# daigo0927/pwcnet

Hardware: AMD Instinct MI355X
Metric: image_pairs_per_sec_448x1024 (higher is better)
Workload: dtype f32 via fp16x2-split MFMA (fp32 tensors and accumulation; big stride-1 convs, level-1 extractor and correlation on the F16 pipe)

## Files before the change

### pwcnet_amd/csrc/conv3x3_h2.hip

```cpp
#pragma once
#include "pwc_common.h"
#include <type_traits>

typedef float pwc_f32x16 __attribute__((ext_vector_type(16)));

struct H2Args {
    const float* x;
    const void* wp;
    const float* bias;
    float* y;
    int x_cs, y_cs;
    int N, H, W;
    int Cin_phys, Cout;
    int apply_act;
    float slope;
    int tiles_x, tiles_y, ncb;
    int dil_y, dil_x;
    int ntiles;
    float* ws_partial;
    unsigned* dbg;
    int Ho, Wo;
    const float* x2;
    int x2_cs, nc16_a;
    const float* x3;
// ... 583 lines not shown
    const H2Geo geo = h2_geometry(H, W, dilation, Cout);
    const int hs = geo.hs, ws = geo.ws;
    const bool filled = nb >= 192 || (nb >= 64 && h2_split_pays(nb, Cin_phys >> 4, h2_cu_count()));
    return hs >= 7 && ws >= 24 && filled && Cin_phys >= 32 ? 1 : 0;
}

#ifdef PWC_HARNESS
static unsigned* h2_debug_counters = nullptr;
#else
constexpr unsigned* h2_debug_counters = nullptr;
#endif

template <int CT, int PT, int WCG, int ABL, int XS = 1, bool S2 = false>
static int h2_launch(H2Args& a, int hs, int ws, float* workspace, size_t workspace_floats, hipStream_t stream) {
    typedef H2Cfg<CT, PT, WCG, XS> C;
    a.tiles_x = (ws + 31) / 32; a.tiles_y = (hs + C::TR - 1) / C::TR; a.ncb = a.Cout / (32 * C::NCT);
    const long nblk = (long)a.N * a.dil_y * a.dil_x * a.tiles_x * a.tiles_y * a.ncb;
    if (nblk * (a.Cin_phys >> 4) >= (1L << 31)) return PWC_ERANGE;
    a.ntiles = (int)nblk;
    const int cus = h2_cu_count();
    int grid = a.ntiles;
    a.ws_partial = nullptr;
    const size_t part = (size_t)C::NCT * 32 * C::TR * 32;
    if (workspace && h2_split_pays(a.ntiles, a.Cin_phys >> 4, cus) && workspace_floats >= (size_t)cus * part) {
        grid = cus;
        a.ws_partial = workspace;
    }
    pwc_allow_dynamic_lds<&conv3x3_h2_kernel<CT, PT, WCG, ABL, XS, S2>>(C::LDS);
    hipLaunchKernelGGL((conv3x3_h2_kernel<CT, PT, WCG, ABL, XS, S2>), dim3((unsigned)grid), dim3(512), C::LDS, stream, a);
    return pwc_launch_status();
}

static bool h2s2_tile_routed(int N, int H, int W, int x_cs, int Cin_phys, int Cout) {
    const bool ok = h2s2_has_tile_image(Cin_phys, Cout) && pwc_conv3x3_s2_tile_admits(N, H, W, x_cs, Cin_phys, Cout);
#ifdef PWC_HARNESS
    if (pwc_conv3x3_s2_tile_debug_mode()) return ok && pwc_conv3x3_s2_tile_debug_mode() > 0;
#endif
    return ok && Cin_phys == 32;
}

template <int ABL = 0>
static int h2_run(const float* x, int x_cs, const float* packed_w, const float* bias, float* y, int y_cs, int N, int H, int W,
                  int Cin_phys, int Cout, int dilation, int apply_act, float slope, pwc_stream_t stream, int variant = 0,
                  float* workspace = nullptr, size_t workspace_floats = 0, int stride = 1, const float* x2 = nullptr, int x2_cs = 0,
                  int Cin_a_phys = 0, uint32_t* status = nullptr, const float* x3 = nullptr, int x3_cs = 0, int Cin_b_phys = 0) {
    if (!x || !packed_w || !bias || !y) return PWC_EINVAL;
    if (x3 && !x2) return PWC_EINVAL;
    const int slack = x3 ? 12 : 0;
    if (x2) {
        const int cb = x3 ? Cin_b_phys : Cin_phys - Cin_a_phys;
        if (Cin_a_phys <= 0 || Cin_a_phys >= Cin_phys || (Cin_a_phys % 16) || x_cs < Cin_a_phys - slack || x2_cs < cb - slack) return PWC_EINVAL;
        if ((x2_cs & 3) || !pwc_aligned16(x2)) return PWC_EALIGN;
        if ((long)H * W * x2_cs * 4 >= (long)PWC_OOB) return PWC_ERANGE;
    }
    if (x3) {
        const int cc = Cin_phys - Cin_a_phys - Cin_b_phys;
        if (Cin_b_phys <= 0 || (Cin_b_phys % 16) || cc <= 0 || x3_cs < cc - 12 || dilation != 1) return PWC_EINVAL;
        if ((x3_cs & 3) || !pwc_aligned16(x3)) return PWC_EALIGN;
        if ((long)H * W * x3_cs * 4 >= (long)PWC_OOB) return PWC_ERANGE;
    }
    if (reinterpret_cast<uintptr_t>(status) & 7u) return PWC_EALIGN;
    if (dilation < 1 || (stride != 1 && stride != 2)) return PWC_EINVAL;
    const bool shape_ok = !(Cin_phys % 16 || Cout % 32 || Cout > H2_MAX_COUT || (stride == 2 && (dilation != 1 || (H & 1) || (W & 1) || x2)));
    if (const int rc = pwc_conv_io_check(x, x_cs, x2 ? Cin_a_phys - slack : Cin_phys, y, y_cs, Cout, packed_w, bias, N, H, W, shape_ok)) return rc;
    if (!pwc_aligned16(workspace)) return PWC_EALIGN;
    if (((long)H * W + W + 2) * x_cs * 4 >= (long)PWC_OOB || (long)H * W * y_cs * 4 >= (long)PWC_OOB) return PWC_ERANGE;
    H2Args a;
    a.x = x; a.wp = packed_w; a.bias = bias; a.y = y; a.x_cs = x_cs; a.y_cs = y_cs;
    a.N = N; a.H = H; a.W = W; a.Cin_phys = Cin_phys; a.Cout = Cout; a.apply_act = apply_act; a.slope = slope;
    const bool s2 = stride == 2;
    a.Ho = s2 ? H / 2 : H; a.Wo = s2 ? W / 2 : W;
    if (s2) a.Cin_phys = 4 * Cin_phys;
    const H2Geo geo = h2_geometry(a.Ho, a.Wo, dilation, Cout);
    a.dil_y = geo.dy; a.dil_x = geo.dx;
    a.dbg = h2_debug_counters;
    a.x2 = x2; a.x2_cs = x2_cs; a.nc16_a = x2 ? Cin_a_phys >> 4 : a.Cin_phys >> 4; a.status = status;
    a.x3 = x3; a.x3_cs = x3_cs; a.nc16_b = x3 ? Cin_b_phys >> 4 : (a.Cin_phys >> 4) - a.nc16_a;
    const int hs = geo.hs, ws = geo.ws;
    if (variant == 0) variant = h2_plan(N, a.Ho, a.Wo, a.Cin_phys, Cout, dilation, nullptr);
    if (variant < 1 || variant > 5) return PWC_EUNSUPPORTED;
    if (Cout % h2_variant(variant).couts) return PWC_EUNSUPPORTED;
    if (s2 && h2s2_tile_routed(N, H, W, x_cs, Cin_phys, Cout))
        return pwc_conv3x3_s2_tile_launch(x, x_cs, packed_w + h2s2_tile_image_offset(Cin_phys, Cout), bias, y, y_cs, N, H, W, Cin_phys,
                                          Cout, apply_act, slope, stream);
    if (s2) {
        switch (variant) {
            case 1: return h2_launch<2, 2, 2, ABL, 1, true>(a, hs, ws, workspace, workspace_floats, (hipStream_t)stream);
            case 2: return h2_launch<2, 2, 1, ABL, 1, true>(a, hs, ws, workspace, workspace_floats, (hipStream_t)stream);
            case 3: return h2_launch<3, 1, 1, ABL, 1, true>(a, hs, ws, workspace, workspace_floats, (hipStream_t)stream);
            case 4: return h2_launch<1, 2, 1, ABL, 1, true>(a, hs, ws, workspace, workspace_floats, (hipStream_t)stream);
            default: return h2_launch<1, 2, 2, ABL, 1, true>(a, hs, ws, workspace, workspace_floats, (hipStream_t)stream);
        }
    }
    if (geo.xs == 2) {
        switch (variant) {
            case 1: return h2_launch<2, 2, 2, ABL, 2>(a, hs, ws, workspace, workspace_floats, (hipStream_t)stream);
            case 3: return h2_launch<3, 1, 1, ABL, 2>(a, hs, ws, workspace, workspace_floats, (hipStream_t)stream);
            case 5: return h2_launch<1, 2, 2, ABL, 2>(a, hs, ws, workspace, workspace_floats, (hipStream_t)stream);
            default: return PWC_EUNSUPPORTED;
        }
    }
    switch (variant) {
        case 1: return h2_launch<2, 2, 2, ABL>(a, hs, ws, workspace, workspace_floats, (hipStream_t)stream);
        case 2: return h2_launch<2, 2, 1, ABL>(a, hs, ws, workspace, workspace_floats, (hipStream_t)stream);
        case 3: return h2_launch<3, 1, 1, ABL>(a, hs, ws, workspace, workspace_floats, (hipStream_t)stream);
        case 4: return h2_launch<1, 2, 1, ABL>(a, hs, ws, workspace, workspace_floats, (hipStream_t)stream);
        default: return h2_launch<1, 2, 2, ABL>(a, hs, ws, workspace, workspace_floats, (hipStream_t)stream);
    }
}

extern "C" size_t pwc_conv3x3_h2_workspace_floats(int N, int H, int W, int Cin_phys, int Cout, int dilation) {
    long nb = 0;
    const int v = h2_plan(N, H, W, Cin_phys, Cout, dilation, &nb);
    const int cus = h2_cu_count();
    if (!v || !h2_split_pays(nb, Cin_phys >> 4, cus)) return 0;
    const H2Variant t = h2_variant(v);
    return (size_t)cus * t.couts * t.rows * 32;
}

extern "C" int pwc_conv3x3_h2_f32(const float* x, int x_cs, const float* packed_w, const float* bias, float* y,
                                  int y_cs, int N, int H, int W, int Cin_phys, int Cout, int dilation,
                                  int apply_act, float slope, float* workspace, size_t workspace_floats, pwc_stream_t stream) {
    return h2_run<0>(x, x_cs, packed_w, bias, y, y_cs, N, H, W, Cin_phys, Cout, dilation, apply_act, slope, stream, 0,
                     workspace, workspace_floats);
}

extern "C" int pwc_conv3x3_h2_ex_f32(const float* x, int x_cs, int Cin_a_phys, const float* x2, int x2_cs,
                                     const float* packed_w, const float* bias, float* y, int y_cs, int N, int H, int W,
                                     int Cin_phys, int Cout, int dilation, int apply_act, float slope, float* workspace,
                                     size_t workspace_floats, uint32_t* status, pwc_stream_t stream) {
    return h2_run<0>(x, x_cs, packed_w, bias, y, y_cs, N, H, W, Cin_phys, Cout, dilation, apply_act, slope, stream, 0,
                     workspace, workspace_floats, 1, x2, x2_cs, Cin_a_phys, status);
}

extern "C" int pwc_conv3x3_h2_ex3_f32(const float* x, int x_cs, int Cin_a_phys, const float* x2, int x2_cs, int Cin_b_phys,
                                      const float* x3, int x3_cs, const float* packed_w, const float* bias, float* y, int y_cs,
                                      int N, int H, int W, int Cin_phys, int Cout, int apply_act, float slope, float* workspace,
                                      size_t workspace_floats, uint32_t* status, pwc_stream_t stream) {
    if (!x2 || !x3) return PWC_EINVAL;
    return h2_run<0>(x, x_cs, packed_w, bias, y, y_cs, N, H, W, Cin_phys, Cout, 1, apply_act, slope, stream, 0,
                     workspace, workspace_floats, 1, x2, x2_cs, Cin_a_phys, status, x3, x3_cs, Cin_b_phys);
}

extern "C" int pwc_conv3x3_h2_stride2_supported(int N, int H, int W, int Cin_phys, int Cout) {
    if (H <= 0 || W <= 0 || (H & 1) || (W & 1) || Cin_phys % 16 || Cin_phys > 32) return 0;
    return pwc_conv3x3_h2_supported(N, H / 2, W / 2, 4 * Cin_phys, Cout, 1);
}

extern "C" size_t pwc_conv3x3_h2_stride2_workspace_floats(int N, int H, int W, int Cin_phys, int Cout) {
    if ((H & 1) || (W & 1)) return 0;
    return pwc_conv3x3_h2_workspace_floats(N, H / 2, W / 2, 4 * Cin_phys, Cout, 1);
}

extern "C" int pwc_conv3x3_h2_stride2_f32(const float* x, int x_cs, const float* packed_w, const float* bias, float* y,
                                          int y_cs, int N, int H, int W, int Cin_phys, int Cout, int apply_act, float slope,
                                          float* workspace, size_t workspace_floats, uint32_t* status, pwc_stream_t stream) {
    return h2_run<0>(x, x_cs, packed_w, bias, y, y_cs, N, H, W, Cin_phys, Cout, 1, apply_act, slope, stream, 0,
                     workspace, workspace_floats, 2, nullptr, 0, 0, status);
}

extern "C" int pwc_conv3x3_h2_plan(int N, int H, int W, int Cin_phys, int Cout, int dilation) {
    return h2_plan(N, H, W, Cin_phys, Cout, dilation, nullptr);
}

extern "C" int pwc_conv3x3_h2_variant_f32(const float* x, int x_cs, const float* packed_w, const float* bias, float* y,
                                          int y_cs, int N, int H, int W, int Cin_phys, int Cout, int dilation,
                                          int apply_act, float slope, int variant, float* workspace, size_t workspace_floats,
// ... 6 lines not shown
```

### pwcnet_amd/csrc/conv3x3_s2.hip

```cpp
#include "pwc_common.h"

typedef unsigned int s2_u32x4 __attribute__((ext_vector_type(4)));
#define S2_OOB 0x80000000u

constexpr int S2_PC = 2 * PWC_S2_TILE_COLS + 1;
constexpr int S2_PR = 2 * PWC_S2_TILE_ROWS + 1;
constexpr int S2_NPX = S2_PR * S2_PC;
constexpr int S2_EVEN = PWC_S2_TILE_COLS + 1;
constexpr int S2_LINE = S2_PC * 32;
constexpr int S2_CC = 64;
constexpr int S2_UB = 5;

struct S2Args {
    const float* x;
    const float* wp;
    const float* bias;
    float* y;
    int x_cs, y_cs;
    int N, H, W, Ho, Wo;
    int Cin_phys, Cout;
    int pad_t, pad_l;
    int apply_act;
    float slope;
    int ntx, nty;
    int cg;
    int nsteps;
};

template <int NBW>
__global__ __launch_bounds__(512) void conv3x3_s2_kernel(const S2Args a) {
    extern __shared__ __attribute__((aligned(16))) char s2_smem[];
    const int t = threadIdx.x, lane = t & 63;
    const int wave = __builtin_amdgcn_readfirstlane(t >> 6);
    int b = blockIdx.x;
    const int tx = b % a.ntx;
    b /= a.ntx;
    const int ty = b % a.nty, n = b / a.nty;

    const __amdgpu_buffer_rsrc_t rx = __builtin_amdgcn_make_buffer_rsrc(
        (void*)a.x, 0, (int)((size_t)a.N * a.H * a.W * a.x_cs * 4), 0x00020000);
    const __amdgpu_buffer_rsrc_t rw = __builtin_amdgcn_make_buffer_rsrc(
        (void*)a.wp, 0, (int)((size_t)a.Cout * a.nsteps * 128), 0x00020000);
    const int m = lane & 15, kq = lane >> 4;
    const int row = wave >> 1, cb0 = (wave & 1) * NBW, nb = a.Cout >> 4;

    f32x4 hh[2][NBW], xx[2][NBW];
#pragma unroll
    for (int hf = 0; hf < 2; ++hf)
#pragma unroll
        for (int j = 0; j < NBW; ++j) {
            hh[hf][j] = f32x4{0.f, 0.f, 0.f, 0.f};
            xx[hf][j] = f32x4{0.f, 0.f, 0.f, 0.f};
        }

    auto fetch_b = [&](s2_u32x4 (&bv)[NBW][2], int s, bool live) {
#pragma unroll
        for (int j = 0; j < NBW; ++j) {
            const int cb = cb0 + j;
            const unsigned vo = (live && cb < nb) ? (unsigned)((cb * a.nsteps + s) * 2048 + lane * 16) : S2_OOB;
            bv[j][0] = __builtin_amdgcn_raw_buffer_load_b128(rw, (int)vo, 0, 0);
            bv[j][1] = __builtin_amdgcn_raw_buffer_load_b128(rw, (int)vo, 1024, 0);
        }
    };

    const int gy0 = 2 * PWC_S2_TILE_ROWS * ty - a.pad_t, gx0 = 2 * PWC_S2_TILE_COLS * tx - a.pad_l;
    for (int c0 = 0; c0 < a.Cin_phys; c0 += S2_CC) {
        const int cc = a.Cin_phys - c0 < S2_CC ? a.Cin_phys - c0 : S2_CC;
        const int cgc = cc >> 5, ng16 = cc >> 4, cqs = 1 + cgc;
        const int nst = 9 * cgc, sbase = c0 >> 5;
        auto gstep = [&](int si) { const int tap = si / cgc; return tap * a.cg + sbase + (si - tap * cgc); };
        if (c0) __syncthreads();
        s2_u32x4 b0[NBW][2], b1[NBW][2];
        fetch_b(b0, gstep(0), true);
        const int nu = S2_NPX << cqs;
#pragma unroll 1
        for (int u0 = t; u0 < nu; u0 += 512 * S2_UB) {
            f32x4 v[S2_UB][2];
            int dst[S2_UB];
#pragma unroll
            for (int k = 0; k < S2_UB; ++k) {
                const int u = u0 + 512 * k;
                const int px = u >> cqs, j = u - (px << cqs);
                const int pr = px / S2_PC, pc = px - pr * S2_PC;
                const int gy = gy0 + pr, gx = gx0 + pc;
                const bool ok = u < nu && (unsigned)gy < (unsigned)a.H && (unsigned)gx < (unsigned)a.W;
                const unsigned vo = ok ? (unsigned)(((n * a.H + gy) * a.W + gx) * a.x_cs + c0 + j * 8) * 4u : S2_OOB;
                v[k][0] = __builtin_bit_cast(f32x4, __builtin_amdgcn_raw_buffer_load_b128(rx, (int)vo, 0, 0));
                v[k][1] = __builtin_bit_cast(f32x4, __builtin_amdgcn_raw_buffer_load_b128(rx, (int)vo, 16, 0));
                const int pos = (pc & 1) ? S2_EVEN + (pc >> 1) : pc >> 1;
                dst[k] = u < nu ? ((pr * ng16 + (j >> 1)) * 2) * S2_LINE + pos * 32 + (j & 1) * 16 : -1;
            }
#pragma unroll
            for (int k = 0; k < S2_UB; ++k)
                if (dst[k] >= 0) {
                    pwc_f16x4 h0, m0, h1, m1;
                    pwc_split4(v[k][0], h0, m0);
                    pwc_split4(v[k][1], h1, m1);
                    *reinterpret_cast<pwc_f16x8*>(s2_smem + dst[k]) = __builtin_shufflevector(h0, h1, 0, 1, 2, 3, 4, 5, 6, 7);
                    *reinterpret_cast<pwc_f16x8*>(s2_smem + dst[k] + S2_LINE) = __builtin_shufflevector(m0, m1, 0, 1, 2, 3, 4, 5, 6, 7);
                }
        }
        __syncthreads();

        auto step = [&](const s2_u32x4 (&bv)[NBW][2], int si) {
            const int tap = si / cgc, c32 = si - tap * cgc;
            const int dy = tap / 3, dx = tap - 3 * dy;
            const int pos = (dx == 1 ? S2_EVEN : 0) + (dx >> 1) + m;
            const char* p = s2_smem + (((2 * row + dy) * ng16 + 2 * c32 + (kq >> 1)) * 2) * S2_LINE + pos * 32 + (kq & 1) * 16;
            pwc_f16x8 ah[2], am[2];
#pragma unroll
            for (int hf = 0; hf < 2; ++hf) {
                ah[hf] = *reinterpret_cast<const pwc_f16x8*>(p + hf * 512);
                am[hf] = *reinterpret_cast<const pwc_f16x8*>(p + hf * 512 + S2_LINE);
            }
#pragma unroll
            for (int j = 0; j < NBW; ++j) {
                const pwc_f16x8 wh = __builtin_bit_cast(pwc_f16x8, bv[j][0]);
                const pwc_f16x8 wm = __builtin_bit_cast(pwc_f16x8, bv[j][1]);
#pragma unroll
                for (int hf = 0; hf < 2; ++hf) {
                    xx[hf][j] = __builtin_amdgcn_mfma_f32_16x16x32_f16(wm, ah[hf], xx[hf][j], 0, 0, 0);
                    hh[hf][j] = __builtin_amdgcn_mfma_f32_16x16x32_f16(wh, ah[hf], hh[hf][j], 0, 0, 0);
                    xx[hf][j] = __builtin_amdgcn_mfma_f32_16x16x32_f16(wh, am[hf], xx[hf][j], 0, 0, 0);
                }
            }
        };
#pragma unroll 1
        for (int si = 0; si < nst; si += 2) {
            fetch_b(b1, gstep(si + 1 < nst ? si + 1 : 0), si + 1 < nst);
            step(b0, si);
            fetch_b(b0, gstep(si + 2 < nst ? si + 2 : 0), si + 2 < nst);
            if (si + 1 < nst) step(b1, si + 1);
        }
    }

    const int oy = PWC_S2_TILE_ROWS * ty + row;
#pragma unroll
    for (int hf = 0; hf < 2; ++hf) {
        const int ox = PWC_S2_TILE_COLS * tx + hf * 16 + m;
        if (oy < a.Ho && ox < a.Wo) {
            float* yp = a.y + ((size_t)(n * a.Ho + oy) * a.Wo + ox) * a.y_cs + 4 * kq;
#pragma unroll
            for (int j = 0; j < NBW; ++j) {
                const int cb = cb0 + j;
                if (cb < nb) {
                    f32x4 v = __builtin_elementwise_fma(xx[hf][j], f32x4{1.f / 2048.f, 1.f / 2048.f, 1.f / 2048.f, 1.f / 2048.f}, hh[hf][j]);
                    v += *reinterpret_cast<const f32x4*>(a.bias + cb * 16 + 4 * kq);
                    if (a.apply_act) v = pwc_lrelu4(v, a.slope);
                    *reinterpret_cast<f32x4*>(yp + cb * 16) = v;
                }
            }
        }
    }
}

template <int NBW>
static int s2_launch(const S2Args& a, hipStream_t s) {
    const long wgs = (long)a.N * a.nty * a.ntx;
    if (wgs >= (1L << 31)) return PWC_ERANGE;
    const int cc = a.Cin_phys < S2_CC ? a.Cin_phys : S2_CC;
    pwc_allow_dynamic_lds<&conv3x3_s2_kernel<NBW>>(S2_NPX * S2_CC * 4);
    hipLaunchKernelGGL((conv3x3_s2_kernel<NBW>), dim3((unsigned)wgs), dim3(512), (size_t)S2_NPX * cc * 4, s, a);
    return pwc_launch_status();
}

bool pwc_conv3x3_s2_tile_admits(int N, int H, int W, int x_cs, int Cin_phys, int Cout) {
    if (N <= 0 || H <= 0 || W <= 0 || Cin_phys <= 0 || Cout <= 0 || x_cs < Cin_phys) return false;
    if (Cin_phys % 32 || Cout % 16 || Cout > 128) return false;
    return pwc_fits_2g(N, H, W, x_cs) && (long)Cout * 9 * (Cin_phys / 32) * 128 < (1L << 31);
}

long pwc_conv3x3_s2_tile_count(int N, int H, int W) {
    const int Ho = (H + 1) / 2, Wo = (W + 1) / 2;
    return (long)N * ((Ho + PWC_S2_TILE_ROWS - 1) / PWC_S2_TILE_ROWS) * ((Wo + PWC_S2_TILE_COLS - 1) / PWC_S2_TILE_COLS);
}

int pwc_conv3x3_s2_tile_launch(const float* x, int x_cs, const float* packed_w, const float* bias, float* y, int y_cs, int N, int H,
                               int W, int Cin_phys, int Cout, int apply_act, float slope, pwc_stream_t stream) {
    if (!pwc_conv3x3_s2_tile_admits(N, H, W, x_cs, Cin_phys, Cout)) return PWC_EUNSUPPORTED;
    S2Args a;
    a.x = x; a.wp = packed_w; a.bias = bias; a.y = y; a.x_cs = x_cs; a.y_cs = y_cs;
    a.N = N; a.H = H; a.W = W;
    pwc_same_pad(H, 2, 1, &a.Ho, &a.pad_t);
    pwc_same_pad(W, 2, 1, &a.Wo, &a.pad_l);
    a.Cin_phys = Cin_phys; a.Cout = Cout; a.apply_act = apply_act; a.slope = slope;
    a.ntx = (a.Wo + PWC_S2_TILE_COLS - 1) / PWC_S2_TILE_COLS;
    a.nty = (a.Ho + PWC_S2_TILE_ROWS - 1) / PWC_S2_TILE_ROWS;
    a.cg = Cin_phys / 32; a.nsteps = 9 * a.cg;
    hipStream_t s = (hipStream_t)stream;
    switch ((Cout / 16 + 1) / 2) {
        case 1: return s2_launch<1>(a, s);
        case 2: return s2_launch<2>(a, s);
        case 3: return s2_launch<3>(a, s);
        default: return s2_launch<4>(a, s);
    }
}

#ifdef PWC_HARNESS
static int s2_tile_mode = 0;
extern "C" int pwc_debug_conv3x3_s2_tile(int mode) { s2_tile_mode = mode; return 0; }
int pwc_conv3x3_s2_tile_debug_mode() { return s2_tile_mode; }
#endif
```

### pwcnet_amd/csrc/conv3x3_sk.hip

```cpp
#include "pwc_common.h"

typedef unsigned int sk_u32x4 __attribute__((ext_vector_type(4)));
#define SK_OOB 0x80000000u

struct SkArgs {
    const float* x;
    const float* wp;
    const float* bias;
    float* y;
    int x_cs, y_cs;
    int N, H, W, Ho, Wo;
    int Cin_phys, Cout;
    int stride, dil, pad_t, pad_l;
    int apply_act;
    float slope;
    int nbx, nby;
    int ntx;
    int nct;
    int cg;
    int nsteps;
};

struct SkTile { int ct, tx, by, n; };
__device__ __forceinline__ SkTile sk_tile(const SkArgs& a) {
// ... 294 lines not shown
    if (Cin_phys % 32 || Cout % 16) return PWC_EUNSUPPORTED;
    if (!pwc_aligned16(packed_w)) return PWC_EALIGN;
    const size_t total = (size_t)9 * Cin_phys * Cout * 2;
    int blocks = (int)((total + 255) / 256);
    if (blocks > 4096) blocks = 4096;
    hipLaunchKernelGGL(conv3x3_sk_pack_kernel, dim3(blocks), dim3(256), 0, (hipStream_t)stream, w_hwio, cin_map, Cin, Cin_phys,
                       Cout, reinterpret_cast<_Float16*>(packed_w));
    return pwc_launch_status();
}

#define PWC_SK_MAX_MACS 100000000L
#define PWC_SK_THIN_MACS 32000000L
#define PWC_SK_LP_MAX_MACS 240000000L
#define PWC_SK_LP_MAX_PIXELS 8192L
#define PWC_SK_S2_MAX_MACS 200000000L
#define PWC_SK_S2_TILE_MIN 192L
extern "C" int pwc_conv3x3_sk_supported(int N, int H, int W, int Cin_phys, int Cout, int stride, int dilation) {
    if (!sk_shape_ok(N, H, W, Cin_phys, Cout, stride, dilation)) return 0;
    int Ho, Wo, pt, pl;
    pwc_same_pad(H, stride, dilation, &Ho, &pt);
    pwc_same_pad(W, stride, dilation, &Wo, &pl);
    if (!pwc_fits_2g(N, H, W, Cin_phys)) return 0;
    const long M = (long)N * Ho * Wo, macs = M * Cin_phys * Cout;
    if (stride == 1 && dilation == 1 && Cin_phys >= 96 && Cin_phys <= 288 && M <= PWC_SK_LP_MAX_PIXELS && macs <= PWC_SK_LP_MAX_MACS)
        return 1;
    if (stride == 2 && dilation == 1 && Cin_phys >= 64 && Cin_phys <= 128 && macs <= PWC_SK_S2_MAX_MACS) return 1;
    if (macs > PWC_SK_MAX_MACS) return 0;
    return (M <= 4096 || stride == 2 || macs <= PWC_SK_THIN_MACS) ? 1 : 0;
}

template <int MT, int NT, int PB>
static int sk_launch(SkArgs a, hipStream_t s) {
    a.ntx = (a.nbx + MT - 1) / MT;
    a.nct = a.Cout / (16 * NT);
    const long wgs = (long)a.N * a.nby * a.ntx * a.nct;
    if (wgs >= (1L << 31)) return PWC_ERANGE;
    hipLaunchKernelGGL((conv3x3_sk_kernel<MT, NT, PB>), dim3((unsigned)wgs), dim3(512), 0, s, a);
    return pwc_launch_status();
}

template <int MT, int NT, int PB, int S>
static int skp_launch(SkArgs a, hipStream_t s) {
    a.ntx = (a.nbx + MT - 1) / MT;
    a.nct = a.Cout / (16 * NT);
    const long wgs = (long)a.N * a.nby * a.ntx * a.nct;
    if (wgs >= (1L << 31)) return PWC_ERANGE;
    constexpr int NPX = (3 * S + 3) * ((4 * MT - 1) * S + 3);
    size_t lds = (size_t)NPX * (a.Cin_phys * 4 + 16);
    if (lds < (size_t)8 * MT * NT * 1024) lds = (size_t)8 * MT * NT * 1024;
    pwc_allow_dynamic_lds<&conv3x3_skp_kernel<MT, NT, PB, S>>(NPX * ((S == 1 ? 288 : 128) * 4 + 16));
    hipLaunchKernelGGL((conv3x3_skp_kernel<MT, NT, PB, S>), dim3((unsigned)wgs), dim3(512), lds, s, a);
    return pwc_launch_status();
}

#ifdef PWC_HARNESS
static int sk_tile_override = 0;
extern "C" int pwc_debug_conv3x3_sk_tile(int tile) { sk_tile_override = tile; return 0; }
#endif

static int sk_run(const float* x, int x_cs, const float* packed_w, const float* bias, float* y, int y_cs,
                  int N, int H, int W, int Cin_phys, int Cout, int stride, int dilation, int apply_act,
                  float slope, int tile_req, pwc_stream_t stream) {
    if (stride < 1 || stride > 2 || dilation < 1) return PWC_EINVAL;
    const bool shape_ok = !(Cin_phys % 32 || Cout % 16);
    if (const int rc = pwc_conv_io_check(x, x_cs, Cin_phys, y, y_cs, Cout, packed_w, bias, N, H, W, shape_ok)) return rc;
    if (!pwc_fits_2g(N, H, W, x_cs)) return PWC_ERANGE;
    SkArgs a;
    a.x = x; a.wp = packed_w; a.bias = bias; a.y = y; a.x_cs = x_cs; a.y_cs = y_cs;
    a.N = N; a.H = H; a.W = W;
    pwc_same_pad(H, stride, dilation, &a.Ho, &a.pad_t);
    pwc_same_pad(W, stride, dilation, &a.Wo, &a.pad_l);
    a.Cin_phys = Cin_phys; a.Cout = Cout; a.stride = stride; a.dil = dilation;
    a.apply_act = apply_act; a.slope = slope;
    a.nbx = (a.Wo + 3) / 4; a.nby = (a.Ho + 3) / 4;
    a.cg = Cin_phys / 32; a.nsteps = 9 * a.cg;
    a.ntx = a.nct = 0;
    const long wgs11 = (long)N * a.nbx * a.nby * (Cout / 16);
    int tile = wgs11 <= 256 ? 11 : (wgs11 <= 1024 || (Cout % 32)) ? 21 : 22;
    const bool lp_ok = dilation == 1 && ((stride == 1 && Cin_phys <= 288) || (stride == 2 && Cin_phys <= 128));
    if (lp_ok && stride == 1 && (Cin_phys >= 192 || (Cin_phys >= 96 && wgs11 > 256)))
        tile = wgs11 <= 256 ? 31 : (wgs11 <= 640 || (Cout % 32)) ? 41 : 42;
    if (lp_ok && stride == 2 && Cin_phys >= 64 && wgs11 > 256) tile = (wgs11 <= 640 || (Cout % 32)) ? 41 : 42;
    const bool s2_ok = stride == 2 && dilation == 1 && pwc_conv3x3_s2_tile_admits(N, H, W, x_cs, Cin_phys, Cout);
    bool s2_tile = tile_req == 50 || (!tile_req && s2_ok && pwc_conv3x3_s2_tile_count(N, H, W) >= PWC_SK_S2_TILE_MIN);
#ifdef PWC_HARNESS
    if (!tile_req && pwc_conv3x3_s2_tile_debug_mode()) s2_tile = s2_ok && pwc_conv3x3_s2_tile_debug_mode() > 0;
#endif
    if (s2_tile) {
        if (!s2_ok) return PWC_EUNSUPPORTED;
        return pwc_conv3x3_s2_tile_launch(x, x_cs, packed_w, bias, y, y_cs, N, H, W, Cin_phys, Cout, apply_act, slope, stream);
    }
    if (tile_req) {
        if (tile_req != 11 && tile_req != 21 && tile_req != 22 && tile_req != 31 && tile_req != 41 && tile_req != 42) return PWC_EINVAL;
        if (((tile_req % 10) == 2 && Cout % 32) || (tile_req > 30 && !lp_ok)) return PWC_EUNSUPPORTED;
        tile = tile_req;
    }
#ifdef PWC_HARNESS
    else if (sk_tile_override && !((sk_tile_override % 10) == 2 && Cout % 32) && !(sk_tile_override > 30 && !lp_ok)) tile = sk_tile_override;
#endif
    hipStream_t s = (hipStream_t)stream;
    switch (tile) {
        case 11: return sk_launch<1, 1, 5>(a, s);
        case 21: return sk_launch<2, 1, 3>(a, s);
        case 22: return sk_launch<2, 2, 2>(a, s);
        case 31: return stride == 1 ? skp_launch<1, 1, 11, 1>(a, s) : skp_launch<1, 1, 11, 2>(a, s);
        case 41: return stride == 1 ? skp_launch<2, 1, 7, 1>(a, s) : skp_launch<2, 1, 7, 2>(a, s);
        default: return stride == 1 ? skp_launch<2, 2, 3, 1>(a, s) : skp_launch<2, 2, 3, 2>(a, s);
    }
}

extern "C" int pwc_conv3x3_sk_f32(const float* x, int x_cs, const float* packed_w, const float* bias, float* y, int y_cs,
                                  int N, int H, int W, int Cin_phys, int Cout, int stride, int dilation, int apply_act,
                                  float slope, pwc_stream_t stream) {
    return sk_run(x, x_cs, packed_w, bias, y, y_cs, N, H, W, Cin_phys, Cout, stride, dilation, apply_act, slope, 0, stream);
}

extern "C" int pwc_conv3x3_sk_variant_f32(const float* x, int x_cs, const float* packed_w, const float* bias, float* y, int y_cs,
                                          int N, int H, int W, int Cin_phys, int Cout, int stride, int dilation, int apply_act,
                                          float slope, int tile, pwc_stream_t stream) {
    if (tile == 0) return PWC_EINVAL;
    return sk_run(x, x_cs, packed_w, bias, y, y_cs, N, H, W, Cin_phys, Cout, stride, dilation, apply_act, slope, tile, stream);
}
```

### pwcnet_amd/csrc/pwc_common.h

```cpp
#pragma once
#include <hip/hip_runtime.h>
#include <stdint.h>

#include "../../include/pwc_hip.h"

typedef float f32x4 __attribute__((ext_vector_type(4)));
typedef float f32x2 __attribute__((ext_vector_type(2)));
typedef _Float16 pwc_f16x8 __attribute__((ext_vector_type(8)));
typedef _Float16 pwc_f16x4 __attribute__((ext_vector_type(4)));
typedef _Float16 pwc_f16x2 __attribute__((ext_vector_type(2)));

#define PWC_WAVE 64

static inline int pwc_launch_status() {
    hipError_t e = hipGetLastError();
    return e == hipSuccess ? PWC_OK : (int)e;
}

template <auto Kernel>
static inline void pwc_allow_dynamic_lds(int bytes) {
    static unsigned long long done[4] = {0, 0, 0, 0};
    int d = 0;
    if (hipGetDevice(&d) == hipSuccess && d >= 0 && d < 256) {
        const unsigned long long bit = 1ull << (d & 63);
// ... 74 lines not shown
__device__ __forceinline__ void pwc_lds_barrier_raw() { asm volatile("s_waitcnt lgkmcnt(0)\n\ts_barrier" ::: "memory"); }
__device__ __forceinline__ void pwc_lds_barrier() {
#if PWC_FENCE_BARRIER
    __builtin_amdgcn_fence(__ATOMIC_RELEASE, "workgroup", "local");
    __builtin_amdgcn_s_barrier();
    __builtin_amdgcn_fence(__ATOMIC_ACQUIRE, "workgroup", "local");
#else
    pwc_lds_barrier_raw();
#endif
}

#define PWC_WAIT_VM(n) __builtin_amdgcn_s_waitcnt(((n) & 15) | (((n) >> 4) << 14) | (7 << 4) | (15 << 8))

__device__ __forceinline__ float pwc_lrelu(float v, float slope) {
    return fmaxf(v, slope * v);
}
__device__ __forceinline__ f32x4 pwc_lrelu4(f32x4 v, float slope) {
    return f32x4{pwc_lrelu(v[0], slope), pwc_lrelu(v[1], slope), pwc_lrelu(v[2], slope), pwc_lrelu(v[3], slope)};
}
__device__ __forceinline__ f32x4 pwc_lrelu4_packed(f32x4 v, float slope) {
    const f32x4 sv = v * slope;
    return f32x4{fmaxf(v[0], sv[0]), fmaxf(v[1], sv[1]), fmaxf(v[2], sv[2]), fmaxf(v[3], sv[3])};
}

__device__ __forceinline__ int pwc_xcd_remap(int b, int nblocks) {
    const int q = nblocks >> 3, r = nblocks & 7;
    const int xcd = b & 7, k = b >> 3;
    const int base = xcd < r ? xcd * (q + 1) : r * (q + 1) + (xcd - r) * q;
    return base + k;
}

__device__ __forceinline__ void pwc_split2(const float x0, const float x1, unsigned& h_pair, unsigned& m_pair) {
    const f32x2 xs = {x0, x1};
    const pwc_f16x2 h2 = __builtin_convertvector(xs, pwc_f16x2);
    const f32x2 xm = xs * 2048.f;
    const unsigned hp = __builtin_bit_cast(unsigned, h2);
    const float neg = -2048.f;
    unsigned mp;
    asm("v_fma_mixlo_f16 %0, %1, %2, %3 op_sel_hi:[1,0,0]" : "=v"(mp) : "v"(hp), "s"(neg), "v"(xm[0]));
    asm("v_fma_mixhi_f16 %0, %1, %2, %3 op_sel:[1,0,0] op_sel_hi:[1,0,0]" : "+v"(mp) : "v"(hp), "s"(neg), "v"(xm[1]));
    h_pair = hp; m_pair = mp;
}
__device__ __forceinline__ void pwc_split4(const f32x4 x, pwc_f16x4& h, pwc_f16x4& m) {
    typedef unsigned u32x2 __attribute__((ext_vector_type(2)));
    u32x2 hp, mp;
    unsigned a, b;
    pwc_split2(x[0], x[1], a, b); hp[0] = a; mp[0] = b;
    pwc_split2(x[2], x[3], a, b); hp[1] = a; mp[1] = b;
    h = __builtin_bit_cast(pwc_f16x4, hp);
    m = __builtin_bit_cast(pwc_f16x4, mp);
}
__device__ __forceinline__ void pwc_split4(const float x0, const float x1, const float x2, const float x3, pwc_f16x4& h, pwc_f16x4& m) {
    pwc_split4(f32x4{x0, x1, x2, x3}, h, m);
}
__device__ __forceinline__ void pwc_split1(const float x, _Float16& h, _Float16& m) {
    h = (_Float16)x;
    m = (_Float16)__builtin_fmaf((float)h, -2048.f, x * 2048.f);
}

template <int COUT = 32>
__global__ void conv3x3_c32_pack_kernel(const float* __restrict__ w, const int32_t* __restrict__ cin_map, int Cin, int Cin_phys,
                                        _Float16* __restrict__ packed) {
    static_assert(COUT == 32, "the row operand of v_mfma_f32_32x32x16_f16");
    const int j16 = Cin_phys >> 4;
    const int total = 9 * j16 * 512;
    for (int idx = blockIdx.x * blockDim.x + threadIdx.x; idx < total; idx += gridDim.x * blockDim.x) {
        const int e = idx & 7, lane = (idx >> 3) & 63;
        const int r = idx >> 9;
        const int j = r % j16, tap = r / j16;
        const int cphys = j * 16 + (lane >> 5) * 8 + e, co = lane & (COUT - 1);
        const int clog = cin_map ? cin_map[cphys] : (cphys < Cin ? cphys : -1);
        float v = 0.f;
        if (clog >= 0 && clog < Cin) v = w[((size_t)tap * Cin + clog) * COUT + co];
        _Float16* dst = packed + (size_t)r * 1024 + lane * 8 + e;
        pwc_split1(v, dst[0], dst[512]);
    }
}

#define PWC_S2_TILE_ROWS 4
#define PWC_S2_TILE_COLS 32
bool pwc_conv3x3_s2_tile_admits(int N, int H, int W, int x_cs, int Cin_phys, int Cout);
long pwc_conv3x3_s2_tile_count(int N, int H, int W);
int pwc_conv3x3_s2_tile_launch(const float* x, int x_cs, const float* packed_w, const float* bias, float* y, int y_cs, int N, int H,
                               int W, int Cin_phys, int Cout, int apply_act, float slope, pwc_stream_t stream);
#ifdef PWC_HARNESS
int pwc_conv3x3_s2_tile_debug_mode();
#endif
```

Baseline: 3543.

## Make stride-2 tile conv persistent with cross-tile prefetch and LDS-resident weights

Rewrites the stride-2 tiled conv as a persistent kernel: a grid capped near CU count loops over tiles and channel chunks, and prefetches the next stage's input patch and weights into registers during the current MFMA loop through a ring of weight buffers. For Cin=32 with Cout<=64, the whole packed weight set is staged once per block in LDS instead of being reloaded from global memory per step. Layers with larger Cin still use the old one-tile-per-block kernel unless a grid cap is requested. The aim is to hide global load latency and cut launch and tail overhead per tile. In exchange it costs more registers and LDS, and the persistent grid may lower occupancy.

```diff
diff --git a/pwcnet_amd/csrc/conv3x3_h2.hip b/pwcnet_amd/csrc/conv3x3_h2.hip
--- a/pwcnet_amd/csrc/conv3x3_h2.hip
+++ b/pwcnet_amd/csrc/conv3x3_h2.hip
@@ -689,7 +689,7 @@
     if (Cout % h2_variant(variant).couts) return PWC_EUNSUPPORTED;
     if (s2 && h2s2_tile_routed(N, H, W, x_cs, Cin_phys, Cout))
         return pwc_conv3x3_s2_tile_launch(x, x_cs, packed_w + h2s2_tile_image_offset(Cin_phys, Cout), bias, y, y_cs, N, H, W, Cin_phys,
-                                          Cout, apply_act, slope, stream);
+                                          Cout, apply_act, slope, 0, stream);
     if (s2) {
         switch (variant) {
             case 1: return h2_launch<2, 2, 2, ABL, 1, true>(a, hs, ws, workspace, workspace_floats, (hipStream_t)stream);
diff --git a/pwcnet_amd/csrc/conv3x3_s2.hip b/pwcnet_amd/csrc/conv3x3_s2.hip
--- a/pwcnet_amd/csrc/conv3x3_s2.hip
+++ b/pwcnet_amd/csrc/conv3x3_s2.hip
@@ -1,7 +1,12 @@
+#include <type_traits>
+
 #include "pwc_common.h"
 
 typedef unsigned int s2_u32x4 __attribute__((ext_vector_type(4)));
 #define S2_OOB 0x80000000u
+#ifndef S2_WLDS_MAX_COUT
+#define S2_WLDS_MAX_COUT 64
+#endif
 
 constexpr int S2_PC = 2 * PWC_S2_TILE_COLS + 1;
 constexpr int S2_PR = 2 * PWC_S2_TILE_ROWS + 1;
@@ -9,7 +14,12 @@
 constexpr int S2_EVEN = PWC_S2_TILE_COLS + 1;
 constexpr int S2_LINE = S2_PC * 32;
 constexpr int S2_CC = 64;
-constexpr int S2_UB = 5;
+#ifndef S2_UB3
+#define S2_UB3 5
+#define S2_UB4 5
+#endif
+constexpr int S2_WLDS_OFF = S2_NPX * 32 * 4;
+constexpr int S2_WLDS_LOADS = S2_WLDS_MAX_COUT ? (S2_WLDS_MAX_COUT * 9 * 128 / 16 + 511) / 512 : 1;
 
 struct S2Args {
     const float* x;
@@ -23,12 +33,23 @@
     int apply_act;
     float slope;
     int ntx, nty;
+    int ntiles;
+    int nch;
     int cg;
     int nsteps;
 };
 
+struct S2Stage {
+    int tile, ch;
+    int n, ty, tx;
+    int gy0, gx0;
+    int c0, cgc;
+};
+
+constexpr int S2_UB1 = 5;
+
 template <int NBW>
-__global__ __launch_bounds__(512) void conv3x3_s2_kernel(const S2Args a) {
+__global__ __launch_bounds__(512) void conv3x3_s2_first_kernel(const S2Args a) {
     extern __shared__ __attribute__((aligned(16))) char s2_smem[];
     const int t = threadIdx.x, lane = t & 63;
     const int wave = __builtin_amdgcn_readfirstlane(t >> 6);
@@ -74,11 +95,11 @@
         fetch_b(b0, gstep(0), true);
         const int nu = S2_NPX << cqs;
 #pragma unroll 1
-        for (int u0 = t; u0 < nu; u0 += 512 * S2_UB) {
-            f32x4 v[S2_UB][2];
-            int dst[S2_UB];
-#pragma unroll
-            for (int k = 0; k < S2_UB; ++k) {
+        for (int u0 = t; u0 < nu; u0 += 512 * S2_UB1) {
+            f32x4 v[S2_UB1][2];
+            int dst[S2_UB1];
+#pragma unroll
+            for (int k = 0; k < S2_UB1; ++k) {
                 const int u = u0 + 512 * k;
                 const int px = u >> cqs, j = u - (px << cqs);
                 const int pr = px / S2_PC, pc = px - pr * S2_PC;
@@ -91,7 +112,7 @@
                 dst[k] = u < nu ? ((pr * ng16 + (j >> 1)) * 2) * S2_LINE + pos * 32 + (j & 1) * 16 : -1;
             }
 #pragma unroll
-            for (int k = 0; k < S2_UB; ++k)
+            for (int k = 0; k < S2_UB1; ++k)
                 if (dst[k] >= 0) {
                     pwc_f16x4 h0, m0, h1, m1;
                     pwc_split4(v[k][0], h0, m0);
@@ -154,13 +175,240 @@
     }
 }
 
+template <int NBW, int UN, bool WLDS, int UB, int RING>
+__global__ __launch_bounds__(512) void conv3x3_s2_kernel(const S2Args a) {
+    extern __shared__ __attribute__((aligned(16))) char s2_smem[];
+    const int t = threadIdx.x, lane = t & 63;
+    const int wave = __builtin_amdgcn_readfirstlane(t >> 6);
+    if ((int)blockIdx.x >= a.ntiles) return;
+
+    const __amdgpu_buffer_rsrc_t rx = __builtin_amdgcn_make_buffer_rsrc(
+        (void*)a.x, 0, (int)((size_t)a.N * a.H * a.W * a.x_cs * 4), 0x00020000);
+    const __amdgpu_buffer_rsrc_t rw = __builtin_amdgcn_make_buffer_rsrc(
+        (void*)a.wp, 0, (int)((size_t)a.Cout * a.nsteps * 128), 0x00020000);
+    const int m = lane & 15, kq = lane >> 4;
+    const int row = wave >> 1, cb0 = (wave & 1) * NBW, nb = a.Cout >> 4;
+
+    f32x4 hh[2][NBW], xx[2][NBW];
+    auto clear = [&]() {
+#pragma unroll
+        for (int hf = 0; hf < 2; ++hf)
+#pragma unroll
+            for (int j = 0; j < NBW; ++j) {
+                hh[hf][j] = f32x4{0.f, 0.f, 0.f, 0.f};
+                xx[hf][j] = f32x4{0.f, 0.f, 0.f, 0.f};
+            }
+    };
+    clear();
+
+    auto stage_at = [&](int tile, int ch) {
+        S2Stage g;
+        g.tile = tile; g.ch = ch;
+        g.tx = tile % a.ntx;
+        const int b = tile / a.ntx;
+        g.ty = b % a.nty; g.n = b / a.nty;
+        g.gy0 = 2 * PWC_S2_TILE_ROWS * g.ty - a.pad_t; g.gx0 = 2 * PWC_S2_TILE_COLS * g.tx - a.pad_l;
+        g.c0 = ch * S2_CC;
+        g.cgc = a.Cin_phys - g.c0 < S2_CC ? 1 : 2;
+        return g;
+    };
+    auto gstep = [&](const S2Stage& g, int si) { const int tap = si / g.cgc; return tap * a.cg + (g.c0 >> 5) + (si - tap * g.cgc); };
+
+    auto fetch_b = [&](s2_u32x4 (&bv)[NBW][2], int s, bool live) {
+#pragma unroll
+        for (int j = 0; j < NBW; ++j) {
+            const int cb = cb0 + j;
+            if constexpr (WLDS) {
+                const char* p = s2_smem + S2_WLDS_OFF + ((cb < nb ? cb : 0) * a.nsteps + s) * 2048 + lane * 16;
+                bv[j][0] = *reinterpret_cast<const s2_u32x4*>(p);
+                bv[j][1] = *reinterpret_cast<const s2_u32x4*>(p + 1024);
+            } else {
+                const unsigned vo = (live && cb < nb) ? (unsigned)((cb * a.nsteps + s) * 2048 + lane * 16) : S2_OOB;
+                bv[j][0] = __builtin_amdgcn_raw_buffer_load_b128(rw, (int)vo, 0, 0);
+                bv[j][1] = __builtin_amdgcn_raw_buffer_load_b128(rw, (int)vo, 1024, 0);
+            }
+        }
+    };
+
+    f32x4 pv[UN][2];
+    auto unit_load = [&](int k, const S2Stage& g, bool live) {
+        const int cqs = 1 + g.cgc, nu = S2_NPX << cqs;
+        const int u = t + 512 * k;
+        const int px = u >> cqs, j = u - (px << cqs);
+        const int pr = px / S2_PC, pc = px - pr * S2_PC;
+        const int gy = g.gy0 + pr, gx = g.gx0 + pc;
+        const bool ok = live && u < nu && (unsigned)gy < (unsigned)a.H && (unsigned)gx < (unsigned)a.W;
+        const unsigned vo = ok ? (unsigned)(((g.n * a.H + gy) * a.W + gx) * a.x_cs + g.c0 + j * 8) * 4u : S2_OOB;
+        pv[k][0] = __builtin_bit_cast(f32x4, __builtin_amdgcn_raw_buffer_load_b128(rx, (int)vo, 0, 0));
+        pv[k][1] = __builtin_bit_cast(f32x4, __builtin_amdgcn_raw_buffer_load_b128(rx, (int)vo, 16, 0));
+    };
+    auto units_write = [&](const S2Stage& g, int k0, int k1) {
+        const int cqs = 1 + g.cgc, nu = S2_NPX << cqs, ng16 = 2 * g.cgc;
+#pragma unroll
+        for (int k = k0; k < k1; ++k) {
+            const int u = t + 512 * k;
+            if (u < nu) {
+                const int px = u >> cqs, j = u - (px << cqs);
+                const int pr = px / S2_PC, pc = px - pr * S2_PC;
+                const int pos = (pc & 1) ? S2_EVEN + (pc >> 1) : pc >> 1;
+                char* dst = s2_smem + ((pr * ng16 + (j >> 1)) * 2) * S2_LINE + pos * 32 + (j & 1) * 16;
+                pwc_f16x4 h0, m0, h1, m1;
+                pwc_split4(pv[k][0], h0, m0);
+                pwc_split4(pv[k][1], h1, m1);
+                *reinterpret_cast<pwc_f16x8*>(dst) = __builtin_shufflevector(h0, h1, 0, 1, 2, 3, 4, 5, 6, 7);
+                *reinterpret_cast<pwc_f16x8*>(dst + S2_LINE) = __builtin_shufflevector(m0, m1, 0, 1, 2, 3, 4, 5, 6, 7);
+            }
+        }
+    };
+
+    auto step = [&](const s2_u32x4 (&bv)[NBW][2], int si, int cgc) {
+        const int ng16 = 2 * cgc;
+        const int tap = si / cgc, c32 = si - tap * cgc;
+        const int dy = tap / 3, dx = tap - 3 * dy;
+        const int pos = (dx == 1 ? S2_EVEN : 0) + (dx >> 1) + m;
+        const char* p = s2_smem + (((2 * row + dy) * ng16 + 2 * c32 + (kq >> 1)) * 2) * S2_LINE + pos * 32 + (kq & 1) * 16;
+        pwc_f16x8 ah[2], am[2];
+#pragma unroll
+        for (int hf = 0; hf < 2; ++hf) {
+            ah[hf] = *reinterpret_cast<const pwc_f16x8*>(p + hf * 512);
+            am[hf] = *reinterpret_cast<const pwc_f16x8*>(p + hf * 512 + S2_LINE);
+        }
+#pragma unroll
+        for (int j = 0; j < NBW; ++j) {
+            const pwc_f16x8 wh = __builtin_bit_cast(pwc_f16x8, bv[j][0]);
+            const pwc_f16x8 wm = __builtin_bit_cast(pwc_f16x8, bv[j][1]);
+#pragma unroll
+            for (int hf = 0; hf < 2; ++hf) {
+                xx[hf][j] = __builtin_amdgcn_mfma_f32_16x16x32_f16(wm, ah[hf], xx[hf][j], 0, 0, 0);
+                hh[hf][j] = __builtin_amdgcn_mfma_f32_16x16x32_f16(wh, ah[hf], hh[hf][j], 0, 0, 0);
+                xx[hf][j] = __builtin_amdgcn_mfma_f32_16x16x32_f16(wh, am[hf], xx[hf][j], 0, 0, 0);
+            }
+        }
+    };
+
+    auto patch = [&](const S2Stage& g) {
+#pragma unroll
+        for (int k0 = 0; k0 < UN; k0 += UB) {
+#pragma unroll
+            for (int k = k0; k < k0 + UB && k < UN; ++k) unit_load(k, g, true);
+            units_write(g, k0, k0 + UB < UN ? k0 + UB : UN);
+        }
+    };
+
+    s2_u32x4 ring[RING][NBW][2];
+    auto kloop = [&](auto cgc_c, const S2Stage& cur, const S2Stage& nxt, bool has_next) {
+        constexpr int CGC = decltype(cgc_c)::value, NST = 9 * CGC, UPS = UB == UN ? (UN + NST - 1) / NST : 0;
+        static_assert(RING == 2 || NST % RING == 0, "the ring slot of a step must not depend on the stage");
+#pragma unroll
+        for (int si = 0; si < NST; ++si) {
+#pragma unroll
+            for (int k = si * UPS; k < si * UPS + UPS; ++k)
+                if (k < UN) unit_load(k, nxt, has_next);
+            const int j = si + RING - 1;
+            if (j < NST) {
+                const int tap = j / CGC;
+                fetch_b(ring[j % RING], tap * a.cg + (cur.c0 >> 5) + (j - tap * CGC), true);
+            } else if constexpr (RING == 3) {
+                fetch_b(ring[j % RING], has_next ? gstep(nxt, j - NST) : 0, has_next);
+            }
+            step(ring[si % RING], si, CGC);
+        }
+    };
+
+    auto epilogue = [&](const S2Stage& g) {
+        const int oy = PWC_S2_TILE_ROWS * g.ty + row;
+#pragma unroll
+        for (int hf = 0; hf < 2; ++hf) {
+            const int ox = PWC_S2_TILE_COLS * g.tx + hf * 16 + m;
+            if (oy < a.Ho && ox < a.Wo) {
+                float* yp = a.y + ((size_t)(g.n * a.Ho + oy) * a.Wo + ox) * a.y_cs + 4 * kq;
+#pragma unroll
+                for (int j = 0; j < NBW; ++j) {
+                    const int cb = cb0 + j;
+                    if (cb < nb) {
+                        f32x4 v = __builtin_elementwise_fma(xx[hf][j], f32x4{1.f / 2048.f, 1.f / 2048.f, 1.f / 2048.f, 1.f / 2048.f}, hh[hf][j]);
+                        v += *reinterpret_cast<const f32x4*>(a.bias + cb * 16 + 4 * kq);
+                        if (a.apply_act) v = pwc_lrelu4(v, a.slope);
+                        *reinterpret_cast<f32x4*>(yp + cb * 16) = v;
+                    }
+                }
+            }
+        }
+    };
+
+    S2Stage cur = stage_at((int)blockIdx.x, 0);
+    if constexpr (!WLDS) {
+#pragma unroll
+        for (int s = 0; s < RING - 1; ++s) fetch_b(ring[s], gstep(cur, s), true);
+    }
+    if constexpr (UB == UN) {
+#pragma unroll
+        for (int k = 0; k < UN; ++k) unit_load(k, cur, true);
+    }
+    if constexpr (WLDS) {
+        const int n16 = a.Cout * a.nsteps * 8;
+        s2_u32x4 wv[S2_WLDS_LOADS];
+#pragma unroll
+        for (int i = 0; i < S2_WLDS_LOADS; ++i) {
+            const int u = t + 512 * i;
+            wv[i] = __builtin_amdgcn_raw_buffer_load_b128(rw, u < n16 ? u * 16 : (int)S2_OOB, 0, 0);
+        }
+#pragma unroll
+        for (int i = 0; i < S2_WLDS_LOADS; ++i) {
+            const int u = t + 512 * i;
+            if (u < n16) *reinterpret_cast<s2_u32x4*>(s2_smem + S2_WLDS_OFF + u * 16) = wv[i];
+        }
+    }
+    if constexpr (UB == UN) units_write(cur, 0, UN);
+    else patch(cur);
+    __syncthreads();
+    if constexpr (WLDS) {
+#pragma unroll
+        for (int s = 0; s < RING - 1; ++s) fetch_b(ring[s], gstep(cur, s), true);
+    }
+
+#pragma unroll 1
+    for (;;) {
+        const bool last_ch = cur.ch + 1 == a.nch;
+        const int ntile = last_ch ? cur.tile + (int)gridDim.x : cur.tile;
+        const bool has_next = ntile < a.ntiles;
+        const S2Stage nxt = stage_at(has_next ? ntile : cur.tile, last_ch ? 0 : cur.ch + 1);
+        if constexpr (UN > 5) {
+            if (cur.cgc == 2) kloop(std::integral_constant<int, 2>{}, cur, nxt, has_next);
+            else kloop(std::integral_constant<int, 1>{}, cur, nxt, has_next);
+        } else {
+            kloop(std::integral_constant<int, 1>{}, cur, nxt, has_next);
+        }
+        if (last_ch) {
+            epilogue(cur);
+            clear();
+        }
+        if (!has_next) break;
+        __syncthreads();
+        if constexpr (RING == 2) fetch_b(ring[0], gstep(nxt, 0), true);
+        if constexpr (UB == UN) units_write(nxt, 0, UN);
+        else patch(nxt);
+        __syncthreads();
+        cur = nxt;
+    }
+}
+
 template <int NBW>
-static int s2_launch(const S2Args& a, hipStream_t s) {
-    const long wgs = (long)a.N * a.nty * a.ntx;
-    if (wgs >= (1L << 31)) return PWC_ERANGE;
+static int s2_launch_first(const S2Args& a, hipStream_t s) {
+    pwc_allow_dynamic_lds<&conv3x3_s2_first_kernel<NBW>>(S2_NPX * S2_CC * 4);
+    hipLaunchKernelGGL((conv3x3_s2_first_kernel<NBW>), dim3((unsigned)a.ntiles), dim3(512), (size_t)S2_NPX * S2_CC * 4, s, a);
+    return pwc_launch_status();
+}
+
+template <int NBW, int UN, bool WLDS, int UB = UN, int RING = 3>
+static int s2_launch(const S2Args& a, int grid_cap, hipStream_t s) {
     const int cc = a.Cin_phys < S2_CC ? a.Cin_phys : S2_CC;
-    pwc_allow_dynamic_lds<&conv3x3_s2_kernel<NBW>>(S2_NPX * S2_CC * 4);
-    hipLaunchKernelGGL((conv3x3_s2_kernel<NBW>), dim3((unsigned)wgs), dim3(512), (size_t)S2_NPX * cc * 4, s, a);
+    const size_t lds = (size_t)S2_NPX * cc * 4 + (WLDS ? (size_t)a.Cout * a.nsteps * 128 : 0);
+    const int per_cu = (UN == 5 && !WLDS && NBW == 1) ? 2 : 1;
+    const long slots = (long)pwc_cu_count() * per_cu;
+    const int grid = grid_cap > 0 ? grid_cap : (int)(a.ntiles < slots ? a.ntiles : slots);
+    pwc_allow_dynamic_lds<&conv3x3_s2_kernel<NBW, UN, WLDS, UB, RING>>(WLDS ? S2_WLDS_OFF + S2_WLDS_MAX_COUT * 9 * 128 : S2_NPX * S2_CC * 4);
+    hipLaunchKernelGGL((conv3x3_s2_kernel<NBW, UN, WLDS, UB, RING>), dim3((unsigned)grid), dim3(512), lds, s, a);
     return pwc_launch_status();
 }
 
@@ -176,7 +424,7 @@
 }
 
 int pwc_conv3x3_s2_tile_launch(const float* x, int x_cs, const float* packed_w, const float* bias, float* y, int y_cs, int N, int H,
-                               int W, int Cin_phys, int Cout, int apply_act, float slope, pwc_stream_t stream) {
+                               int W, int Cin_phys, int Cout, int apply_act, float slope, int grid_cap, pwc_stream_t stream) {
     if (!pwc_conv3x3_s2_tile_admits(N, H, W, x_cs, Cin_phys, Cout)) return PWC_EUNSUPPORTED;
     S2Args a;
     a.x = x; a.wp = packed_w; a.bias = bias; a.y = y; a.x_cs = x_cs; a.y_cs = y_cs;
@@ -186,13 +434,35 @@
     a.Cin_phys = Cin_phys; a.Cout = Cout; a.apply_act = apply_act; a.slope = slope;
     a.ntx = (a.Wo + PWC_S2_TILE_COLS - 1) / PWC_S2_TILE_COLS;
     a.nty = (a.Ho + PWC_S2_TILE_ROWS - 1) / PWC_S2_TILE_ROWS;
+    const long ntiles = (long)N * a.nty * a.ntx;
+    if (ntiles >= (1L << 31)) return PWC_ERANGE;
+    a.ntiles = (int)ntiles;
+    a.nch = (Cin_phys + S2_CC - 1) / S2_CC;
     a.cg = Cin_phys / 32; a.nsteps = 9 * a.cg;
     hipStream_t s = (hipStream_t)stream;
-    switch ((Cout / 16 + 1) / 2) {
-        case 1: return s2_launch<1>(a, s);
-        case 2: return s2_launch<2>(a, s);
-        case 3: return s2_launch<3>(a, s);
-        default: return s2_launch<4>(a, s);
+    const int nbw = (Cout / 16 + 1) / 2;
+    if (Cin_phys == 32 && Cout <= S2_WLDS_MAX_COUT) return nbw == 1 ? s2_launch<1, 5, true>(a, grid_cap, s) : s2_launch<2, 5, true>(a, grid_cap, s);
+    if (Cin_phys == 32) {
+        switch (nbw) {
+            case 1: return s2_launch<1, 5, false>(a, grid_cap, s);
+            case 2: return s2_launch<2, 5, false>(a, grid_cap, s);
+            case 3: return s2_launch<3, 5, false>(a, grid_cap, s);
+            default: return s2_launch<4, 5, false>(a, grid_cap, s);
+        }
+    }
+    if (grid_cap <= 0) {
+        switch (nbw) {
+            case 1: return s2_launch_first<1>(a, s);
+            case 2: return s2_launch_first<2>(a, s);
+            case 3: return s2_launch_first<3>(a, s);
+            default: return s2_launch_first<4>(a, s);
+        }
+    }
+    switch (nbw) {
+        case 1: return s2_launch<1, 10, false>(a, grid_cap, s);
+        case 2: return s2_launch<2, 10, false>(a, grid_cap, s);
+        case 3: return s2_launch<3, 10, false, S2_UB3>(a, grid_cap, s);
+        default: return s2_launch<4, 10, false, S2_UB4, 2>(a, grid_cap, s);
     }
 }
 
diff --git a/pwcnet_amd/csrc/conv3x3_sk.hip b/pwcnet_amd/csrc/conv3x3_sk.hip
--- a/pwcnet_amd/csrc/conv3x3_sk.hip
+++ b/pwcnet_amd/csrc/conv3x3_sk.hip
@@ -400,13 +400,14 @@
         tile = wgs11 <= 256 ? 31 : (wgs11 <= 640 || (Cout % 32)) ? 41 : 42;
     if (lp_ok && stride == 2 && Cin_phys >= 64 && wgs11 > 256) tile = (wgs11 <= 640 || (Cout % 32)) ? 41 : 42;
     const bool s2_ok = stride == 2 && dilation == 1 && pwc_conv3x3_s2_tile_admits(N, H, W, x_cs, Cin_phys, Cout);
-    bool s2_tile = tile_req == 50 || (!tile_req && s2_ok && pwc_conv3x3_s2_tile_count(N, H, W) >= PWC_SK_S2_TILE_MIN);
+    bool s2_tile = (tile_req >= 50 && tile_req <= 52) || (!tile_req && s2_ok && pwc_conv3x3_s2_tile_count(N, H, W) >= PWC_SK_S2_TILE_MIN);
 #ifdef PWC_HARNESS
     if (!tile_req && pwc_conv3x3_s2_tile_debug_mode()) s2_tile = s2_ok && pwc_conv3x3_s2_tile_debug_mode() > 0;
 #endif
     if (s2_tile) {
         if (!s2_ok) return PWC_EUNSUPPORTED;
-        return pwc_conv3x3_s2_tile_launch(x, x_cs, packed_w, bias, y, y_cs, N, H, W, Cin_phys, Cout, apply_act, slope, stream);
+        return pwc_conv3x3_s2_tile_launch(x, x_cs, packed_w, bias, y, y_cs, N, H, W, Cin_phys, Cout, apply_act, slope,
+                                          tile_req > 50 ? tile_req - 50 : 0, stream);
     }
     if (tile_req) {
         if (tile_req != 11 && tile_req != 21 && tile_req != 22 && tile_req != 31 && tile_req != 41 && tile_req != 42) return PWC_EINVAL;
diff --git a/pwcnet_amd/csrc/pwc_common.h b/pwcnet_amd/csrc/pwc_common.h
--- a/pwcnet_amd/csrc/pwc_common.h
+++ b/pwcnet_amd/csrc/pwc_common.h
@@ -180,7 +180,7 @@
 bool pwc_conv3x3_s2_tile_admits(int N, int H, int W, int x_cs, int Cin_phys, int Cout);
 long pwc_conv3x3_s2_tile_count(int N, int H, int W);
 int pwc_conv3x3_s2_tile_launch(const float* x, int x_cs, const float* packed_w, const float* bias, float* y, int y_cs, int N, int H,
-                               int W, int Cin_phys, int Cout, int apply_act, float slope, pwc_stream_t stream);
+                               int W, int Cin_phys, int Cout, int apply_act, float slope, int grid_cap, pwc_stream_t stream);
 #ifdef PWC_HARNESS
 int pwc_conv3x3_s2_tile_debug_mode();
 #endif
```

After: 3541. Within noise of the previous version (-0.1%).
